# sz3/libcimbar

Measured on AMD Instinct MI355X. Metric: decoded cimbar frames/s (1024x1024 mode-B), higher is better.
Workload: dtype u8; 1 GPU; BASELINE configs[1]: 1024 clean mode-B frames per GPU per step, device-resident, bit-exact; distinct_input_batches=4, exchange_ranks=1, parallelism=frame-sharded x1; 3 steps in flight (pipelined entry point)

## Files before the change

### libcimbar_amd/csrc/cimbar_hip.hip

```cpp
#include <hip/hip_runtime.h>
#include <type_traits>

#include <cfloat>
#include <climits>
#include <cmath>
#include <cstdint>
#include <cstdio>
#include <cstdlib>
#include <cstring>
#include <memory>
#include <mutex>
#include <string>
#include <utility>
#include <vector>

#include "../../include/cimbar_hip.h"

#include "devbuf.hip.inc"

#include "deliver.hip.inc"

#define CIMBAR_MODE 68
#define CIMBAR_NS m68
#include "mode.hip.inc"
#undef CIMBAR_MODE
#undef CIMBAR_NS
#define CIMBAR_MODE 67
#define CIMBAR_NS m67
#include "mode.hip.inc"
#undef CIMBAR_MODE
#undef CIMBAR_NS
#define CIMBAR_MODE 66
#define CIMBAR_NS m66
#include "mode.hip.inc"
#undef CIMBAR_MODE
#undef CIMBAR_NS
#define CIMBAR_MODE 4
#define CIMBAR_NS m4
#include "mode.hip.inc"
#undef CIMBAR_MODE
#undef CIMBAR_NS
#define CIMBAR_MODE 8
#define CIMBAR_NS m8
#include "mode.hip.inc"
#undef CIMBAR_MODE
#undef CIMBAR_NS

#include "api.hip.inc"
#include "automode.hip.inc"
#include "comm.hip.inc"
#include "png.hip.inc"
```

### libcimbar_amd/csrc/k2_symbols.hip.inc

```
__device__ __forceinline__ void window_rows(const uint32_t* __restrict__ plane, int x0, int y0, uint32_t rows[10])
{
	const int j = x0 >> 5, sh = 54 - (x0 & 31);
	const int j1 = j + 1 > 31 ? 31 : j + 1;
#pragma unroll
	for (int i = 0; i < 10; ++i) {
		const uint32_t* r = plane + (size_t)(y0 + i) * PLANE_ROW;
		uint64_t v = ((uint64_t)r[j] << 32) | r[j1];
		rows[i] = (uint32_t)(v >> sh) & 0x3FFu;
	}
}

__device__ __forceinline__ uint64_t window_hash(const uint32_t rows[10], int w)
{
	const int cs = 2 - (w % 3), r0 = w / 3;
	uint64_t h = 0;
#pragma unroll
	for (int k = 0; k < 8; ++k) h = (h << 8) | ((rows[r0 + k] >> cs) & 0xFFu);
	return h;
}

__device__ __forceinline__ uint32_t best_tile(uint64_t h)
{
	uint32_t best = 0xFFFFu;
#pragma unroll
	for (int t = 0; t < 16; ++t) {
		uint32_t d = (uint32_t)__popcll(h ^ c_tile[t]);
		uint32_t key = (d << 4) | (uint32_t)t;
		best = key < best ? key : best;
	}
	return best;
}

__device__ __forceinline__ bool is_seed(int i)
{
	return i == 0 || i == TOP_W - 1 || i == NCELLS - 1 || i == NCELLS - TOP_W || i == TOP_CELLS || i == TOP_CELLS + DIM_X - 1 ||
	       i == NCELLS - 1 - TOP_CELLS || i == NCELLS - TOP_CELLS - DIM_X;
}

constexpr uint32_t TILE_SLOT_MUL = 0x61b91u;
__constant__ uint8_t c_tile_slot[32];
__device__ __forceinline__ uint32_t exact_tile(uint64_t h)
{
	const uint32_t slot = c_tile_slot[(((uint32_t)h ^ (uint32_t)(h >> 32)) * TILE_SLOT_MUL) >> 27];
	return (slot < 16 && c_tile[slot] == h) ? slot : 16u;
}

__device__ __forceinline__ void window_rows_lds(const uint32_t* rows32, int x0, uint32_t rows[10])
{
	const int j = x0 >> 5, sh = 54 - (x0 & 31);
	const int j1 = j + 1 > 31 ? 31 : j + 1;
#pragma unroll
	for (int i = 0; i < 10; ++i) {
		const uint32_t* r = rows32 + i * 32;
		uint64_t v = ((uint64_t)r[j] << 32) | r[j1];
		rows[i] = (uint32_t)(v >> sh) & 0x3FFu;
	}
}

__device__ __forceinline__ int cell_index(int row, int col)
{
	if (row >= DIM_Y) return -1;
	const bool margin = row < MARKER || row >= DIM_Y - MARKER;
	if (margin && (col < MARKER || col >= DIM_X - MARKER)) return -1;
	if (row < MARKER) return row * TOP_W + (col - MARKER);
	if (row < DIM_Y - MARKER) return TOP_CELLS + (row - MARKER) * DIM_X + col;
	return TOP_CELLS + MID_CELLS + (row - (DIM_Y - MARKER)) * TOP_W + (col - MARKER);
}

constexpr int K2_ROWS = 8, K2_STRIPS = (DIM_Y + K2_ROWS - 1) / K2_ROWS, K2_BLOCKS = (K2_STRIPS + 3) / 4, K2_WORDS = IMG_W / 32;
static_assert(K2_ROWS % 2 == 0 && IMG_W % 32 == 0, "cell rows are processed in pairs; a bit row is whole words");
__global__ __launch_bounds__(256) void k_symbols(const uint32_t* __restrict__ plane, Tables tb, uint8_t* __restrict__ symbols,
                                                 uint32_t* __restrict__ flood_flag, int f0)
{
	__shared__ uint16_t s_queue[4][K2_ROWS * DIM_X];
	__shared__ uint64_t s_tile[16];
	__shared__ uint8_t s_slot[32];
	if (threadIdx.x < 16) s_tile[threadIdx.x] = c_tile[threadIdx.x];
	if (threadIdx.x < 32) s_slot[threadIdx.x] = c_tile_slot[threadIdx.x];
	__syncthreads();
	const int lane = threadIdx.x & 63, wave = __builtin_amdgcn_readfirstlane((int)(threadIdx.x >> 6));
	const int strip = blockIdx.x * 4 + wave;
	if (strip >= K2_STRIPS) return;
	const int f = f0 + blockIdx.y;
	const uint32_t* pl = plane + (size_t)f * PLANE_WORDS;
	uint8_t* sym = symbols + (size_t)f * NCELLS;
	uint16_t* queue = s_queue[wave];
	int qn = 0;
	const unsigned long long below = (1ull << lane) - 1ull;
	const int w = lane & 31, half = lane >> 5;
	const int c0 = w == 0 ? 0 : (32 * w - OFFSET + PITCH - 1) / PITCH;

	for (int rr = 0; rr < K2_ROWS; rr += 2) {
		const int row = strip * K2_ROWS + rr + half;
		if (strip * K2_ROWS + rr >= DIM_Y) break;
		const bool row_ok = row < DIM_Y && w < K2_WORDS;
		const uint32_t* r = pl + (size_t)(OFFSET + (row < DIM_Y ? row : DIM_Y - 1) * PITCH) * PLANE_ROW + w;
		uint32_t own[8];
#pragma unroll
		for (int k = 0; k < 8; ++k) own[k] = r[k * PLANE_ROW];
		uint64_t V[8];
#pragma unroll
		for (int k = 0; k < 8; ++k) V[k] = ((uint64_t)own[k] << 32) | from_right_lane(own[k], 0u);
#pragma unroll
		for (int q = 0; q < 4; ++q) {
			const int col = c0 + q;
			const int x0 = OFFSET + col * PITCH;
			const int i = (row_ok && col < DIM_X && (x0 >> 5) == w) ? cell_index(row, col) : -1;
			const int sh = 56 - (x0 & 31);
			uint32_t hi = 0, lo = 0;
#pragma unroll
			for (int k = 0; k < 4; ++k) {
				hi = (hi << 8) | ((uint32_t)(V[k] >> sh) & 0xFFu);
				lo = (lo << 8) | ((uint32_t)(V[k + 4] >> sh) & 0xFFu);
			}
			const uint32_t slot = s_slot[((lo ^ hi) * TILE_SLOT_MUL) >> 27];
			const uint64_t cand_tile = s_tile[slot & 15u];
			const bool exact = slot < 16 && cand_tile == (((uint64_t)hi << 32) | lo);
			if (i >= 0 && exact) sym[i] = (uint8_t)slot;
			const unsigned long long qm = __builtin_amdgcn_ballot_w64(i >= 0 && !exact);
			if (i >= 0 && !exact) queue[qn + (int)__popcll(qm & below)] = (uint16_t)((rr + half) * DIM_X + col);
			qn += (int)__popcll(qm);
		}
	}
	__builtin_amdgcn_fence(__ATOMIC_RELEASE, "wavefront");
	__builtin_amdgcn_wave_barrier();
	__builtin_amdgcn_s_waitcnt(0);

	bool shifted = false;
	for (int q = lane; q < qn; q += 64) {
		const int lc = queue[q];
		const int row = strip * K2_ROWS + lc / DIM_X, col = lc % DIM_X;
		const int i = cell_index(row, col);
		uint32_t rows[10];
		window_rows(pl, OFFSET + col * PITCH - 1, OFFSET + row * PITCH - 1, rows);
		const uint32_t centre = best_tile(window_hash(rows, 4));
		const uint32_t dc = centre >> 4;
		sym[i] = (uint8_t)(centre & 15u);
		if (dc != 0) {
			uint32_t other = 0xFFFFu;
			const int side[4] = {5, 7, 3, 1};
#pragma unroll
			for (int k = 0; k < 4; ++k) { uint32_t bt = best_tile(window_hash(rows, side[k])); other = bt < other ? bt : other; }
			if (is_seed(i)) {
				const int corner[4] = {8, 0, 2, 6};
#pragma unroll
				for (int k = 0; k < 4; ++k) { uint32_t bt = best_tile(window_hash(rows, corner[k])); other = bt < other ? bt : other; }
			}
			shifted |= (other >> 4) < dc;
		}
	}
	if (shifted) atomicOr(&flood_flag[f], 1u);
}
```

Measured before the change: 1.392 million frames/s.

## Rewrite symbol-hash extraction with perm/alignbit and precomputed per-lane cell masks

The exact-match fast path in k_symbols now builds each cell's 64-bit window hash from byte permutes (v_perm) and alignbit on the lane's own word plus a DPP-fetched neighbour word, instead of 64-bit shifts and per-byte packing. Cell validity and indices are precomputed per lane as bitmasks and row bases, so cell_index is no longer called per cell. Queueing of inexact cells uses mbcnt and is skipped entirely when the wave has no misses. The aim is fewer VALU instructions in the hot loop, at the cost of relying on static assumptions about PITCH and OFFSET alignment and a reversed cell order within each word.

```diff
diff --git a/libcimbar_amd/csrc/cimbar_hip.hip b/libcimbar_amd/csrc/cimbar_hip.hip
--- a/libcimbar_amd/csrc/cimbar_hip.hip
+++ b/libcimbar_amd/csrc/cimbar_hip.hip
@@ -19,6 +19,14 @@
 #include "devbuf.hip.inc"
 
 #include "deliver.hip.inc"
+
+namespace {
+template <bool TOP>
+__device__ __forceinline__ uint32_t gather4(uint32_t a, uint32_t b, uint32_t c, uint32_t d)
+{
+	return __builtin_amdgcn_perm(a, b, TOP ? 0x07030c0cu : 0x04000c0cu) | __builtin_amdgcn_perm(c, d, TOP ? 0x0c0c0703u : 0x0c0c0400u);
+}
+}
 
 #define CIMBAR_MODE 68
 #define CIMBAR_NS m68
diff --git a/libcimbar_amd/csrc/k2_symbols.hip.inc b/libcimbar_amd/csrc/k2_symbols.hip.inc
--- a/libcimbar_amd/csrc/k2_symbols.hip.inc
+++ b/libcimbar_amd/csrc/k2_symbols.hip.inc
@@ -69,6 +69,8 @@
 
 constexpr int K2_ROWS = 8, K2_STRIPS = (DIM_Y + K2_ROWS - 1) / K2_ROWS, K2_BLOCKS = (K2_STRIPS + 3) / 4, K2_WORDS = IMG_W / 32;
 static_assert(K2_ROWS % 2 == 0 && IMG_W % 32 == 0, "cell rows are processed in pairs; a bit row is whole words");
+static_assert(4 * PITCH >= 32 && 31 - PITCH + 8 <= 32, "at most four cells start in a word, and only the last of them can leave it");
+static_assert((OFFSET + (DIM_X - 1) * PITCH) % 32 != 0, "the last cell that starts in a word never starts at the word's bit 0 (the alignbit shift would be 32)");
 __global__ __launch_bounds__(256) void k_symbols(const uint32_t* __restrict__ plane, Tables tb, uint8_t* __restrict__ symbols,
                                                  uint32_t* __restrict__ flood_flag, int f0)
 {
@@ -86,40 +88,64 @@
 	uint8_t* sym = symbols + (size_t)f * NCELLS;
 	uint16_t* queue = s_queue[wave];
 	int qn = 0;
-	const unsigned long long below = (1ull << lane) - 1ull;
 	const int w = lane & 31, half = lane >> 5;
 	const int c0 = w == 0 ? 0 : (32 * w - OFFSET + PITCH - 1) / PITCH;
+	const int c1e = (32 * (w + 1) - OFFSET + PITCH - 1) / PITCH, c1 = c1e < DIM_X ? c1e : DIM_X;
+	const int ncell = w < K2_WORDS && c1 > c0 ? c1 - c0 : 0, cl = c1 - 1;
+	const uint32_t vmask_all = (1u << ncell) - 1u;
+	uint32_t vmask_mid = 0;
+#pragma unroll
+	for (int q = 0; q < 4; ++q) vmask_mid |= (q < ncell && cl - q >= MARKER && cl - q < DIM_X - MARKER) ? 1u << q : 0u;
+	const uint32_t p0 = (uint32_t)(OFFSET + cl * PITCH) & 31u;
+	uint32_t shq[4];
+	shq[0] = (32u - p0) & 31u;
+#pragma unroll
+	for (int q = 1; q < 4; ++q) shq[q] = (24u - p0 + (uint32_t)(PITCH * q)) & 31u;
 
 	for (int rr = 0; rr < K2_ROWS; rr += 2) {
 		const int row = strip * K2_ROWS + rr + half;
 		if (strip * K2_ROWS + rr >= DIM_Y) break;
-		const bool row_ok = row < DIM_Y && w < K2_WORDS;
 		const uint32_t* r = pl + (size_t)(OFFSET + (row < DIM_Y ? row : DIM_Y - 1) * PITCH) * PLANE_ROW + w;
-		uint32_t own[8];
+		uint32_t own[8], right[8];
 #pragma unroll
 		for (int k = 0; k < 8; ++k) own[k] = r[k * PLANE_ROW];
-		uint64_t V[8];
 #pragma unroll
-		for (int k = 0; k < 8; ++k) V[k] = ((uint64_t)own[k] << 32) | from_right_lane(own[k], 0u);
+		for (int k = 0; k < 8; ++k) right[k] = (uint32_t)__builtin_amdgcn_update_dpp(0, (int)own[k], 0x130, 0xf, 0xf, true);
+		const bool top = row < MARKER, bottom = row >= DIM_Y - MARKER;
+		const int rowbase = top ? row * TOP_W - MARKER
+		                        : bottom ? TOP_CELLS + MID_CELLS + (row - (DIM_Y - MARKER)) * TOP_W - MARKER : TOP_CELLS + (row - MARKER) * DIM_X;
+		const uint32_t vm = row >= DIM_Y ? 0u : (top || bottom) ? vmask_mid : vmask_all;
+		uint32_t hi[4], lo[4], slot[4];
+		uint64_t cand_tile[4];
 #pragma unroll
 		for (int q = 0; q < 4; ++q) {
-			const int col = c0 + q;
-			const int x0 = OFFSET + col * PITCH;
-			const int i = (row_ok && col < DIM_X && (x0 >> 5) == w) ? cell_index(row, col) : -1;
-			const int sh = 56 - (x0 & 31);
-			uint32_t hi = 0, lo = 0;
+			uint32_t b[8];
 #pragma unroll
-			for (int k = 0; k < 4; ++k) {
-				hi = (hi << 8) | ((uint32_t)(V[k] >> sh) & 0xFFu);
-				lo = (lo << 8) | ((uint32_t)(V[k + 4] >> sh) & 0xFFu);
+			for (int k = 0; k < 8; ++k) b[k] = q == 0 ? __builtin_amdgcn_alignbit(own[k], right[k], shq[0]) : own[k] >> shq[q];
+			hi[q] = q == 0 ? gather4<true>(b[0], b[1], b[2], b[3]) : gather4<false>(b[0], b[1], b[2], b[3]);
+			lo[q] = q == 0 ? gather4<true>(b[4], b[5], b[6], b[7]) : gather4<false>(b[4], b[5], b[6], b[7]);
+		}
+#pragma unroll
+		for (int q = 0; q < 4; ++q) slot[q] = s_slot[((lo[q] ^ hi[q]) * TILE_SLOT_MUL) >> 27];
+#pragma unroll
+		for (int q = 0; q < 4; ++q) cand_tile[q] = s_tile[slot[q] & 15u];
+		uint32_t inexact = 0;
+#pragma unroll
+		for (int q = 0; q < 4; ++q) {
+			const bool valid = (vm >> q) & 1u;
+			const bool exact = (slot[q] < 16) & (cand_tile[q] == (((uint64_t)hi[q] << 32) | lo[q]));
+			if (valid & exact) sym[rowbase + cl - q] = (uint8_t)slot[q];
+			inexact |= (valid & !exact) ? 1u << q : 0u;
+		}
+		if (__builtin_amdgcn_ballot_w64(inexact != 0) != 0ull) {
+#pragma unroll
+			for (int q = 0; q < 4; ++q) {
+				const bool push = (inexact >> q) & 1u;
+				const unsigned long long qm = __builtin_amdgcn_ballot_w64(push);
+				const uint32_t at = __builtin_amdgcn_mbcnt_hi((uint32_t)(qm >> 32), __builtin_amdgcn_mbcnt_lo((uint32_t)qm, (uint32_t)qn));
+				if (push) queue[at] = (uint16_t)((rr + half) * DIM_X + cl - q);
+				qn += (int)__popcll(qm);
 			}
-			const uint32_t slot = s_slot[((lo ^ hi) * TILE_SLOT_MUL) >> 27];
-			const uint64_t cand_tile = s_tile[slot & 15u];
-			const bool exact = slot < 16 && cand_tile == (((uint64_t)hi << 32) | lo);
-			if (i >= 0 && exact) sym[i] = (uint8_t)slot;
-			const unsigned long long qm = __builtin_amdgcn_ballot_w64(i >= 0 && !exact);
-			if (i >= 0 && !exact) queue[qn + (int)__popcll(qm & below)] = (uint16_t)((rr + half) * DIM_X + col);
-			qn += (int)__popcll(qm);
 		}
 	}
 	__builtin_amdgcn_fence(__ATOMIC_RELEASE, "wavefront");
```

Result: no change. 1.399 million frames/s, median of 2 (+0.5%).
